# QCDIS/KaFKA-InferenceEngine

Hardware: AMD Instinct MI355X
Metric: pixel-state updates/sec (whole node), 10980^2 S2 tile, 7-param state (higher is better)
Workload: dtype fp32

## Files before the change

csrc/kf_bindings.cpp:

```cpp
#include <pybind11/pybind11.h>
#include <pybind11/stl.h>
#include <stdexcept>
#include <string>
#include <vector>
#include "kf_launch.h"
#include "kf_deflate.h"
#include "kf_inflate.h"
#include "kf_stream.h"

namespace py = pybind11;
using namespace kf;
namespace kf {
void bind_tiff(py::module_& m);
}

template <typename T>
static T* P(uintptr_t v) { return reinterpret_cast<T*>(v); }

static void check_hip(hipError_t e, const char* what) {
  if (e != hipSuccess) throw std::runtime_error(std::string(what) + ": " + hipGetErrorString(e));
}
static void check_host(int rc, const char* what) {
  if (rc != 0) throw std::runtime_error(std::string(what) + ": unsupported n_params on host runner");
}
// ... 87 lines not shown
      .PTR_FIELD(AnalysisArgs, a_out, float*)
      .PTR_FIELD(AnalysisArgs, b_out, float*)
      .PTR_FIELD(AnalysisArgs, a_in, const float*)
      .PTR_FIELD(AnalysisArgs, b_in, const float*)
      .PTR_FIELD(AnalysisArgs, status, uint8_t*)
      .PTR_FIELD(AnalysisArgs, partials, double*)
      .PTR_FIELD(AnalysisArgs, partials_first, double*)
      .PTR_FIELD(AnalysisArgs, order, const int32_t*)
      .def_readwrite("n_visit", &AnalysisArgs::n_visit)
      .PTR_FIELD(AnalysisArgs, n_visit_dev, const int32_t*)
      .PTR_FIELD(AnalysisArgs, dn_out, float*)
      .def_readwrite("a_rows", &AnalysisArgs::a_rows)
      .def_readwrite("dom_check", &AnalysisArgs::dom_check)
      .ARR_FIELD(AnalysisArgs, dom_lo, float)
      .ARR_FIELD(AnalysisArgs, dom_hi, float)
      .def_readwrite("gn_fused", &AnalysisArgs::gn_fused)
      .def_readwrite("band_layout", &AnalysisArgs::band_layout)
      .PTR_FIELD(AnalysisArgs, prop, const PropArgs*)
      .PTR_FIELD(AnalysisArgs, out_mean, float*)
      .PTR_FIELD(AnalysisArgs, out_unc, float*)
      .PTR_FIELD(AnalysisArgs, out_idx, const int64_t*)
      .def_readwrite("out_plane", &AnalysisArgs::out_plane)
      .def_readwrite("reg_gamma", &AnalysisArgs::reg_gamma)
      .def_readwrite("reg_mask", &AnalysisArgs::reg_mask)
      .PTR_FIELD(AnalysisArgs, reg_nbr, const int32_t*)
      .PTR_FIELD(AnalysisArgs, reg_v, float*)
      .PTR_FIELD(AnalysisArgs, x0_out, float*)
      .PTR_FIELD(AnalysisArgs, line_tab, const float*)
      .def_readwrite("line_t0", &AnalysisArgs::line_t0)
      .def_readwrite("line_inv_h", &AnalysisArgs::line_inv_h)
      .def_readwrite("line_n", &AnalysisArgs::line_n)
      .def_readwrite("line_j", &AnalysisArgs::line_j)
      .def_readwrite("a_struct", &AnalysisArgs::a_struct)
      .GEO_FIELDS(AnalysisArgs, reg_geo);

  py::class_<GainArgs>(m, "GainArgs")
      .def(py::init([]() { GainArgs a; memset(&a, 0, sizeof(a)); return a; }))
      .def_readwrite("N", &GainArgs::N)
      .def_readwrite("ld", &GainArgs::ld)
      .def_readwrite("n_bands", &GainArgs::n_bands)
      .def_readwrite("joseph", &GainArgs::joseph)
      .def_readwrite("fast_d", &GainArgs::fast_d)
      .def_readwrite("fast_obs", &GainArgs::fast_obs)
      .def_readwrite("out_plane", &GainArgs::out_plane)
      .def_readwrite("gpm_frags", &GainArgs::gpm_frags)
      .def_readwrite("gpm_global", &GainArgs::gpm_global)
      .def_readwrite("band_layout", &GainArgs::band_layout)
      .def_readwrite("split_mixlo", &GainArgs::split_mixlo)
      .def_readwrite("gn_fused", &GainArgs::gn_fused)
      .def_readwrite("n_visit", &GainArgs::n_visit)
      .PTR_FIELD(GainArgs, n_visit_dev, const int32_t*)
      .def_readwrite("pdiag_rows", &GainArgs::pdiag_rows)
      .PTR_FIELD(GainArgs, partials_first, double*)
      .PTR_FIELD(GainArgs, line_tab, const float*)
      .def_readwrite("line_t0", &GainArgs::line_t0)
      .def_readwrite("line_inv_h", &GainArgs::line_inv_h)
      .def_readwrite("line_n", &GainArgs::line_n)
      .def_readwrite("line_j", &GainArgs::line_j)
      .PTR_FIELD(GainArgs, order, const int32_t*)
      .PTR_FIELD(GainArgs, dn_out, float*)
      .PTR_FIELD(GainArgs, prop, const PropArgs*)
      .PTR_FIELD(GainArgs, out_mean, float*)
      .PTR_FIELD(GainArgs, out_unc, float*)
      .PTR_FIELD(GainArgs, out_idx, const int64_t*)
      .PTR_FIELD(GainArgs, bands, const BandDesc*)
      .PTR_FIELD(GainArgs, x_prev, const float*)
      .PTR_FIELD(GainArgs, x_f, const float*)
// ... 390 lines not shown
```

csrc/kf_core.h:

```cpp
#pragma once
#include <stdint.h>
#include <math.h>

#if defined(__HIPCC__)
#include <hip/hip_runtime.h>
#define KF_HD __host__ __device__ __forceinline__
#else
#define KF_HD inline __attribute__((always_inline))
#endif

enum : int {
  KF_PH_PROLOGUE = 0,
  KF_PH_FORECAST = 1,
  KF_PH_BAND_IN = 2,
  KF_PH_GP = 3,
  KF_PH_BAND_OUT = 4,
  KF_PH_SOLVE = 5,
  KF_PH_GROUPS = 6,
  KF_PH_NSLOT = 8
};
#if defined(KF_PHASE_CLOCKS) && defined(__HIPCC__)
static __device__ unsigned long long kf_phase_clk[KF_PH_NSLOT];
#endif
#if defined(KF_PHASE_CLOCKS) && defined(__HIP_DEVICE_COMPILE__)
// ... 161 lines not shown

KF_HD int32_t geo_neighbour(const StripGeo& g, int64_t N, int64_t p, int k) {
  const uint32_t w = (uint32_t)g.w;
  const uint32_t r = (uint32_t)p / w, c = (uint32_t)p - r * w;
  switch (k) {
    case 0: return r > 0 ? (int32_t)(p - w) : ((g.halo & 1) ? (int32_t)(N + c) : -1);
    case 1: return r + 1 < (uint32_t)g.h ? (int32_t)(p + w) : ((g.halo & 2) ? (int32_t)(N + g.n_up + c) : -1);
    case 2: return c > 0 ? (int32_t)(p - 1) : -1;
    default: return c + 1 < w ? (int32_t)(p + 1) : -1;
  }
}

constexpr int SPEC_ANY = 0, SPEC_PROP = 1, SPEC_PROP_REG = 2;
constexpr int SPEC_PROP_PF = 3;
constexpr int SPEC_PROP_TIP = 4, SPEC_PROP_REG_TIP = 5, SPEC_PROP_PF_TIP = 6;
KF_HD constexpr bool spec_sparse(int spec) { return spec >= SPEC_PROP_TIP; }
KF_HD constexpr int spec_base(int spec) { return spec_sparse(spec) ? spec - 3 : spec; }
constexpr int A_STRUCT_TIP = 1, A_STRUCT_TIP_PRIOR = 2;
template <int SPEC>
struct SpecMask { typedef StructDense type; };
template <> struct SpecMask<SPEC_PROP_TIP> { typedef StructTip type; };
template <> struct SpecMask<SPEC_PROP_REG_TIP> { typedef StructTip type; };
template <> struct SpecMask<SPEC_PROP_PF_TIP> { typedef StructTip type; };

enum AnalysisVariant : int32_t {
  AV_DEFAULT = 0,
  AV_VALU_ORACLE = 4,
  AV_GT_PREFETCH = 7,
  AV_RUNTIME_LAYOUT = 10,
  AV_PER_BAND_OPERAND = 14,
  AV_BLOCK_ORDER = 16,
  AV_GENERIC_SPEC = 18,
  AV_DENSE_SOLVE = 20,
  AV_MIXLO_SPLIT = 22
};

struct AnalysisArgs {
  int64_t N, ld;
  int32_t n_bands, solve;
  int32_t fast_d, fast_obs;
  int32_t variant;
  int32_t gpm_frags;
  int32_t gpm_global;
  const BandDesc* bands;
  const float* x_prev;
  const float* x_f;
  const float* pf_inv;
  float* x_out;
  float* a_out;
  float* b_out;
  const float* a_in;
  const float* b_in;
  uint8_t* status;
  double* partials;
  const PropArgs* prop;
  float* out_mean;
  float* out_unc;
  const int64_t* out_idx;
  int64_t out_plane;
  float reg_gamma;
  uint32_t reg_mask;
  const int32_t* reg_nbr;
  float* reg_v;
  float* x0_out;
  StripGeo reg_geo;
  int32_t gn_fused;
  int32_t band_layout;
  double* partials_first;
  const int32_t* order;
  int64_t n_visit;
  const int32_t* n_visit_dev;
  float* dn_out;
  uint64_t a_rows;
  int32_t dom_check;
  float dom_lo[MAX_D];
  float dom_hi[MAX_D];
  const float* line_tab;
  float line_t0, line_inv_h;
  int32_t line_n, line_j;
  int32_t a_struct;
};

KF_HD int64_t visit_bounded(int64_t n_visit, int64_t N, const int32_t* n_dev) {
  const int64_t n = n_visit > 0 ? n_visit : N;
  if (!n_dev) return n;
  const int64_t d = *n_dev;
  return d < 0 ? 0 : (d < n ? d : n);
}
KF_HD int64_t visit_count(const AnalysisArgs& a) { return visit_bounded(a.n_visit, a.N, a.n_visit_dev); }

template <int NP, typename AP>
KF_HD bool state_out_of_domain(AP a, const float (&x)[NP]) {
  if (!a->dom_check) return false;
  bool o = false;
#pragma unroll
  for (int j = 0; j < NP; ++j) o = o || !(x[j] >= a->dom_lo[j] && x[j] <= a->dom_hi[j]);
  return o;
}
KF_HD bool a_row_on(uint64_t rows, int t) { return rows == 0 || ((rows >> t) & 1u); }



KF_HD int64_t visit_px(const int32_t* order, int64_t q) { return order ? (int64_t)order[q] : q; }
template <int NP>
KF_HD float gather_state(const float (&x)[NP], int idx) {
  float v = x[0];
#pragma unroll
  for (int j = 1; j < NP; ++j) v = (idx == j) ? x[j] : v;
  return v;
}

template <int NP>
KF_HD float gather_state_u(const float (&x)[NP], int idx) {
  float v = x[0];
// ... 1866 lines not shown
```

csrc/kf_device.h:

```cpp
#pragma once
#include <hip/hip_runtime.h>
#include "kf_core.h"
#include "kf_launch.h"
#include "kf_gp_mfma.h"

namespace kf {

constexpr int BLOCK = 256;

__device__ __forceinline__ double wave_sum(double v) {
#pragma unroll
  for (int off = 32; off > 0; off >>= 1) v += __shfl_xor(v, off, 64);
  return v;
}

template <int BS = BLOCK>
__device__ __forceinline__ void block_partial(double v, double* partials) {
  __shared__ double red[BS / 64];
  v = wave_sum(v);
  const int lane = threadIdx.x & 63, wid = threadIdx.x >> 6;
  if (lane == 0) red[wid] = v;
  __syncthreads();
  if (threadIdx.x == 0) {
    double s = 0.0;
// ... 110 lines not shown
  } else {
    for (int64_t base = (int64_t)blockIdx.x * BS + (threadIdx.x - lane); base < nv; base += stride) {
      const int64_t q = base + lane;
      const bool act = q < nv;
      const int64_t p = visit_px(a.order, act ? q : nv - 1);
      float dn1;
      const float dn = pixel_analysis_mfma<NP, D, FOBS, false, false, LAYOUT, IL, SPEC, MIXLO>(a, p, act, gpm_lds,
                                                                                              dn1 KF_PHASE_ARG);
      {
        float* dno = opaque((const KF_CONST_AS AnalysisArgs*)__builtin_amdgcn_kernarg_segment_ptr())->dn_out;
        if (act && dno) KF_PX(dno, 0, p) = dn;
      }
      acc += act ? (double)dn : 0.0;
      acc1 += act ? (double)dn1 : 0.0;
    }
  }
  analysis_partials<BS>(a, acc, acc1);
  KF_PHASE_KERNEL_END
#endif
}

template <int NP, int D, int FOBS, int BS = BLOCK, int MINW = 1, int LAYOUT = BAND_LAYOUT_RUNTIME, bool IL = false,
          int SPEC = SPEC_ANY>
__global__ __launch_bounds__(BS, MINW) void analysis_mfma_kernel(AnalysisArgs a) {
  analysis_mfma_body<NP, D, FOBS, BS, LAYOUT, IL, SPEC, false>(a);
}

template <int NP, int D, int FOBS, int BS = BLOCK, int MINW = 1, int LAYOUT = BAND_LAYOUT_RUNTIME, bool IL = false,
          int SPEC = SPEC_ANY>
__global__ __launch_bounds__(BS, MINW) void analysis_mfma_mixlo_kernel(AnalysisArgs a) {
  analysis_mfma_body<NP, D, FOBS, BS, LAYOUT, IL, SPEC, true>(a);
}

template <int NP, int D, int FOBS, bool PF, bool IL, int SPEC, bool MIXLO>
__device__ __forceinline__ void analysis_mfma_g_body(const AnalysisArgs& a) {
  static_assert(BLOCK / 64 == GPM_G_WAVES, "per-wave LDS transpose buffers of gp_mfma_sums_g_xb");
#if defined(__HIP_DEVICE_COMPILE__)
  KF_PHASE_KERNEL_BEGIN
  double acc = 0.0, acc1 = 0.0;
  const int lane = threadIdx.x & 63;
  const int64_t stride = (int64_t)gridDim.x * BLOCK;
  const int64_t nv = visit_count(a);
  for (int64_t base = (int64_t)blockIdx.x * BLOCK + (threadIdx.x - lane); base < nv; base += stride) {
    const int64_t q = base + lane;
    const bool act = q < nv;
    const int64_t p = visit_px(a.order, act ? q : nv - 1);
    float dn1;
    const float dn = pixel_analysis_mfma<NP, D, FOBS, true, PF, BAND_LAYOUT_RUNTIME, IL, SPEC, MIXLO>(
        a, p, act, nullptr, dn1 KF_PHASE_ARG);
    {
      float* dno = opaque((const KF_CONST_AS AnalysisArgs*)__builtin_amdgcn_kernarg_segment_ptr())->dn_out;
      if (act && dno) KF_PX(dno, 0, p) = dn;
    }
    acc += act ? (double)dn : 0.0;
    acc1 += act ? (double)dn1 : 0.0;
  }
  analysis_partials(a, acc, acc1);
  KF_PHASE_KERNEL_END
#endif
}

template <int NP, int D, int FOBS, bool PF = false, bool IL = false, int SPEC = SPEC_ANY>
__global__ __launch_bounds__(BLOCK, 2) void analysis_mfma_g_kernel(AnalysisArgs a) {
  analysis_mfma_g_body<NP, D, FOBS, PF, IL, SPEC, false>(a);
}

// ... 359 lines not shown
  }
#define KF_MFMA_GO(OBS_, BS_, MINW_, LAY_)                                   \
  {                                                                         \
    if (gpm_il_default<NP, LAY_>() != (a.variant == AV_BLOCK_ORDER))        \
      KF_MFMA_GO1(OBS_, BS_, MINW_, LAY_, true, SPEC_ANY)                   \
    else KF_MFMA_GO1(OBS_, BS_, MINW_, LAY_, false, SPEC_ANY)               \
  }
#define KF_MFMA_GO_SPEC(OBS_, BS_, MINW_, LAY_)                                                      \
  {                                                                                                 \
    constexpr bool IL_ = gpm_il_default<NP, LAY_>();                                                \
    const bool tips = (a.a_struct & A_STRUCT_TIP) && a.variant != AV_DENSE_SOLVE;                   \
    if (a.variant == AV_MIXLO_SPLIT) {     \
      if (!a.prop) KF_MFMA_GO1M(OBS_, BS_, MINW_, LAY_, IL_, SPEC_ANY)                              \
      else if (small) KF_MFMA_GO1M(OBS_, BS_, MINW_, LAY_, IL_, SPEC_PROP_PF_TIP)                   \
      else KF_MFMA_GO1M(OBS_, BS_, MINW_, LAY_, IL_, SPEC_PROP_TIP)                                 \
    }                                                                                               \
    else if (!a.prop || a.variant == AV_BLOCK_ORDER || a.variant == AV_GENERIC_SPEC)                \
      KF_MFMA_GO(OBS_, BS_, MINW_, LAY_)                                                            \
    else if (a.reg_v && tips) KF_MFMA_GO1(OBS_, BS_, MINW_, LAY_, IL_, SPEC_PROP_REG_TIP)          \
    else if (a.reg_v) KF_MFMA_GO1(OBS_, BS_, MINW_, LAY_, IL_, SPEC_PROP_REG)                      \
    else if (small && tips) KF_MFMA_GO1(OBS_, BS_, MINW_, LAY_, IL_, SPEC_PROP_PF_TIP)              \
    else if (small) KF_MFMA_GO1(OBS_, BS_, MINW_, LAY_, IL_, SPEC_PROP_PF)                          \
    else if (tips) KF_MFMA_GO1(OBS_, BS_, MINW_, LAY_, IL_, SPEC_PROP_TIP)                          \
    else KF_MFMA_GO1(OBS_, BS_, MINW_, LAY_, IL_, SPEC_PROP)                                        \
  }
      constexpr int MW = NP <= 7 ? 3 : 1;
      bool tip = false;
      const bool small = a.gpm_frags <= 4 * a.n_bands * gpm_frags_per_chunk(FD) + 1;
      (void)small;
      if constexpr (NP == 7 && FD == 4)
        tip = a.band_layout == BAND_LAYOUT_TIP && a.n_bands == 2 && a.variant != AV_RUNTIME_LAYOUT;
      if (a.fast_obs == OBS_DN16) {
        if constexpr (NP == 7 && FD == 4) {
          if (tip) {
            KF_MFMA_GO_SPEC(OBS_DN16, BLOCK, 3, BAND_LAYOUT_TIP)
            return true;
          }
        }
        KF_MFMA_GO(OBS_DN16, BLOCK, MW, BAND_LAYOUT_RUNTIME)
      } else if (a.fast_obs == OBS_F32) {
        if constexpr (NP == 7 && FD == 4) {
          if (tip) {
            KF_MFMA_GO(OBS_F32, BLOCK, 3, BAND_LAYOUT_TIP)
            return true;
          }
        }
        KF_MFMA_GO(OBS_F32, BLOCK, MW, BAND_LAYOUT_RUNTIME)
      } else {
        return false;
      }
#undef KF_MFMA_GO_SPEC
#undef KF_MFMA_GO
#undef KF_MFMA_GO1
#undef KF_MFMA_GO1M
      return true;
    }
    if constexpr (FD == NP && NP >= 7) {
      if (a.gpm_global && a.variant != AV_VALU_ORACLE) {
        constexpr bool IL = gpm_il_default<NP, BAND_LAYOUT_RUNTIME>();
        if (a.fast_obs == OBS_DN16 && a.variant == AV_GT_PREFETCH)
          launch_tiles(analysis_mfma_g_kernel<NP, FD, OBS_DN16, true>, BLOCK, 0, a, grid, s, n_part);
        else if (NP == 10 && a.fast_obs == OBS_DN16 && a.variant == AV_MIXLO_SPLIT && a.prop && !a.reg_v) {
          if constexpr (NP == 10)
            launch_tiles(analysis_mfma_g_mixlo_kernel<NP, FD, OBS_DN16, false, true, SPEC_PROP>, BLOCK, 0, a, grid, s,
                         n_part);
        } else if (NP == 10 && a.fast_obs == OBS_DN16 && a.variant == AV_MIXLO_SPLIT) {
// ... 60 lines not shown
```

csrc/kf_gp_mfma.h:

```cpp
#pragma once
#include <hip/hip_runtime.h>
#include <type_traits>
#include "kf_core.h"

namespace kf {

typedef _Float16 kf_h8 __attribute__((ext_vector_type(8)));
typedef float kf_f16v __attribute__((ext_vector_type(16)));
typedef uint32_t kf_u4 __attribute__((ext_vector_type(4)));
typedef __fp16 kf_hp2 __attribute__((ext_vector_type(2)));

KF_HD constexpr int gpm_k_steps(int D) { return (3 * D + 2 + 15) / 16; }
KF_HD constexpr int gpm_lo_row(int D) { return D + 1 <= 8 ? 8 : 16; }
KF_HD constexpr int gpm_sum_rows(int D) { return 2 * (D + 1); }
KF_HD constexpr int gpm_frags_per_chunk(int D) { return 64 * gpm_k_steps(D) + 4 * gpm_sum_rows(D); }
constexpr int GPM_MAX_D = 10;
constexpr int GPM_MAX_BANDS = 4;
constexpr int GPM_G_WAVES = 4;

#if defined(__HIP_DEVICE_COMPILE__)
__device__ __forceinline__ uint32_t gpm_pack(_Float16 a, _Float16 b) {
  return (uint32_t)__builtin_bit_cast(uint16_t, a) | ((uint32_t)__builtin_bit_cast(uint16_t, b) << 16);
}

// ... 649 lines not shown
          if (ka->a_out) store_a_rows<NP, M>(ka, p, A);
#pragma unroll
          for (int j = 0; j < NP; ++j) KF_PXS(ka->x_out, j * ld, p) = x1[j];
          if (ka->out_unc) {
            const int64_t r = ka->out_idx ? KF_PXS(ka->out_idx, 0, p) : p;
            const int64_t pl = ka->out_plane;
            if (ka->out_mean) {
#pragma unroll
              for (int j = 0; j < NP; ++j) KF_PXS(ka->out_mean, j * pl, r) = x1[j];
            }
#pragma unroll
            for (int j = 0; j < NP; ++j) KF_PXS(ka->out_unc, j * pl, r) = kf_rsqrt(A[tri(NP, j, j)]);
          }
          if (ka->status) KF_PXS(ka->status, 0, p) = st;
        }
        KF_PHASE(KF_PH_SOLVE)
        return 0.f;
      }
    }
  }
  if (!SPARSE || it + 1 >= ka->gn_fused) {
    if (state_out_of_domain<NP>(ka, x0)) st |= ST_OUT_OF_DOMAIN;
  }
  const bool last = it + 1 >= ka->gn_fused;
  const float dn = analysis_epilogue<NP, true, SPEC>(ka, p, A, b, x0, st, last && act, last);
  KF_PHASE(KF_PH_SOLVE)
  if (last) return act ? dn : 0.f;
  dn_first = dn;
#pragma unroll
  for (int j = 0; j < NP; ++j) x0[j] = b[j];
  }
}

template <int NP, int D, int FOBS, bool GT = false, bool IL = false, bool MIXLO = false>
__device__ __forceinline__ float pixel_gain_mfma(const GainArgs& a, int64_t p, bool act, const kf_h8* lds,
                                                 float& dn1) {
  constexpr bool SXC = GT && D == NP && D % 2 == 0;
  kf_h8 sxb[2][gpm_k_steps(D)];
  int sx_it = -1;
  return gain_pixel<NP>(a, p, act, dn1, [&](int bi, int it, const float (&x0)[NP], float& y, float& w, float& H0,
                                            float (&h)[NP], bool& ok) -> bool {
    int off = 0;
    if constexpr (!GT)
      for (int bj = 0; bj < bi; ++bj) off += cptr(a.bands)[bj].gpm_nchunk * gpm_frags_per_chunk(D);
    const KF_CONST_AS BandDesc* bdp = cptr(a.bands) + bi;
    decode_obs<FOBS>(*bdp, p, y, w);
    const bool use = act && (w > 0.f);
    H0 = 0.f;
#pragma unroll
    for (int j = 0; j < NP; ++j) h[j] = 0.f;
    ok = false;
    const int nch = bdp->gpm_nchunk;
    bool tabled = false;
    const KF_CONST_AS GainArgs* la = opaque((const KF_CONST_AS GainArgs*)__builtin_amdgcn_kernarg_segment_ptr());
    if (it == 0 && !a.x_prev && la->line_tab && __any(use)) {
      const LinePos lp = line_pos<NP>(la, x0, a.n_bands * (D + 1) * 4);
      if (__all(lp.in || !use)) {
        float g[D];
        line_eval<D>(lp.row + bi * (D + 1) * 4, lp.s, H0, g);
        const KF_CONST_AS BandDesc* q = opaque(bdp);
        if (q->map_identity) {
#pragma unroll
          for (int d = 0; d < D && d < NP; ++d) h[d] = g[d];
        } else {
#pragma unroll
          for (int d = 0; d < D; ++d) {
// ... 57 lines not shown
```

kafka_inferenceengine_amd/ops/kernels.py:

```python
from __future__ import annotations

import itertools
from dataclasses import dataclass
from enum import IntEnum

import numpy as np
import torch

from ..models.gp import gpm_frags_per_chunk
from ..utils.blocks import ntri
from . import _ext

OBS_NONE, OBS_F32, OBS_DN16, OBS_BF16, OBS_BF16Y = 0, 1, 2, 3, 4
ST_NONSPD, ST_NONFINITE, ST_BAD_OP, ST_NO_OBS, ST_FALLBACK, ST_OUT_OF_DOMAIN = 1, 2, 4, 8, 16, 32
SUPPORTED_NP = (1, 2, 3, 4, 7, 10)


def ext():
    return _ext.require_ext()


def _ptr(t):
    return 0 if t is None else int(t.data_ptr())

# ... 57 lines not shown

def check_np(n_params: int):
    if n_params not in SUPPORTED_NP:
        raise ValueError(f"n_params={n_params} has no compiled kernel (supported: {SUPPORTED_NP}); "
                         "pad the state (engine.padding) to a supported size")


def grid_for(N: int) -> int:
    return int(ext().grid(int(N)))


def partials_buffer(N: int, device) -> torch.Tensor:
    return torch.zeros(grid_for(N), dtype=torch.float64, device=device)


def _set_valid(partials, n):
    if partials is not None:
        partials._kf_n = int(n)


@dataclass
class BandTable:
    buf: torch.Tensor
    n: int
    keepalive: tuple
    fast_d: int = 0
    fast_obs: int = 0
    gpm_frags: int = 0
    gpm_global: bool = False
    layout: int = 0
    dom: tuple | None = None
    specs: tuple = ()
    tip_maps: bool = False

    @property
    def ptr(self) -> int:
        return int(self.buf.data_ptr())


OP_PRECOMP = 0
OP_LINEAR = 1
OP_GP = 2


GPM_MAX_LDS = 160 * 1024
GPM_MAX_BANDS = 4
GPM_GLOBAL_D = (7, 10)
GAIN_GLOBAL_D = (10,)

BAND_LAYOUT_TIP = 1
BAND_LAYOUT_SHARED_X = 2
FD_PRECOMP = -1
FD_LINEAR = -2


class Variant(IntEnum):
    DEFAULT = 0
    VALU_ORACLE = 4
    GT_PREFETCH = 7
    RUNTIME_LAYOUT = 10
    PER_BAND_OPERAND = 14
    BLOCK_ORDER = 16
    GENERIC_SPEC = 18
    DENSE_SOLVE = 20
    MIXLO_SPLIT = 22


DEFAULT_VARIANT = Variant.DEFAULT


class _PinnedRing:

    SLOT = 16 << 10
    SLOTS = 64

    def __init__(self, device):
        self.device = device
        self.buf = torch.empty(self.SLOT * self.SLOTS, dtype=torch.uint8, pin_memory=True)
        self.events = [None] * self.SLOTS
        self.i = 0

    def copy(self, cpu: torch.Tensor) -> torch.Tensor:
        n = cpu.numel() * cpu.element_size()
        j = self.i
        self.i = (self.i + 1) % self.SLOTS
        if self.events[j] is not None:
            self.events[j].synchronize()
        stage = self.buf[j * self.SLOT:j * self.SLOT + n]
        stage.copy_(cpu.reshape(-1).view(torch.uint8))
        out = torch.empty(n, dtype=torch.uint8, device=self.device)
        out.copy_(stage, non_blocking=True)
        ev = torch.cuda.Event()
        ev.record(torch.cuda.current_stream(self.device))
        self.events[j] = ev
        return out.view(cpu.dtype).view(cpu.shape)


_RINGS = {}
# ... 12 lines not shown
        return ring.copy(cpu)
    return cpu.pin_memory().to(device, non_blocking=True)


def make_band_table(descs: list, device, keepalive=(), specs=()) -> BandTable:
    raw = ext().pack_band_descs(descs)
    cpu = torch.frombuffer(bytearray(raw), dtype=torch.uint8) if raw else torch.zeros(8, dtype=torch.uint8)
    buf = small_h2d(cpu, device)
    fast_d = fast_obs = 0
    obs = {d.obs for d in descs}
    one_obs = next(iter(obs)) if len(obs) == 1 else None
    if descs and all(d.op == OP_GP for d in descs):
        ds = {d.d for d in descs}
        if len(ds) == 1 and one_obs in (OBS_F32, OBS_DN16):
            fast_d, fast_obs = next(iter(ds)), one_obs
    elif descs and one_obs in (OBS_F32, OBS_DN16, OBS_BF16, OBS_BF16Y) and all(d.op == OP_PRECOMP for d in descs):
        fast_d, fast_obs = FD_PRECOMP, one_obs
    elif descs and one_obs in (OBS_F32, OBS_DN16, OBS_BF16, OBS_BF16Y) and all(d.op == OP_LINEAR for d in descs):
        fast_d, fast_obs = FD_LINEAR, one_obs
    gpm_frags, gpm_global = 0, False
    if fast_d > 0 and all(d.gpm_nchunk > 0 for d in descs):
        gpm_frags = sum(d.gpm_nchunk for d in descs) * gpm_frags_per_chunk(fast_d) + 1
        if gpm_frags * 16 > GPM_MAX_LDS or len(descs) > GPM_MAX_BANDS:
            gpm_frags, gpm_global = 0, fast_d in GPM_GLOBAL_D
    layout = 0
    if fast_d == 4 and gpm_frags > 0 and [d.map_kind for d in descs] == [2, 3]:
        layout = BAND_LAYOUT_TIP
    elif (gpm_global and fast_d % 2 == 0 and all(d.map_identity for d in descs)
          and len({tuple(d.center[:fast_d]) for d in descs}) == 1):
        layout = BAND_LAYOUT_SHARED_X
    tip_maps = len(descs) == 2 and all(d.op == OP_GP and d.d == 4 for d in descs) and \
        [d.map_kind for d in descs] == [2, 3]
    return BandTable(buf, len(descs), tuple(keepalive), fast_d, fast_obs, gpm_frags, gpm_global, layout,
                     _state_domain(descs), tuple(specs), tip_maps)


def _state_domain(descs):
    lo, hi, any_ = [-np.inf] * 16, [np.inf] * 16, False
    for d in descs:
        if d.op != OP_GP or not d.dom_check:
            continue
        m, c, dl, dh = d.map, d.center, d.dom_lo, d.dom_hi
        for i in range(int(d.d)):
            j = int(m[i])
            lo[j] = max(lo[j], float(dl[i]) + float(c[i]))
            hi[j] = min(hi[j], float(dh[i]) + float(c[i]))
            any_ = True
    return (lo, hi) if any_ else None


LINE_TABLES = True
_LINE_CACHE: dict = {}


def _prop_single(mask: int):
    mask = int(mask)
    if mask == 0:
        return -1
    return mask.bit_length() - 1 if mask & (mask - 1) == 0 else None


def line_fields(bands: BandTable, prop, n_params: int, dev):
    if dev.type != "cuda" or prop is None or bands.fast_d <= 0 or not bands.specs or \
            not (bands.gpm_frags > 0 or bands.gpm_global):
        return None
    if any(getattr(sp, "kind", None) != OP_GP or len(sp.state_map) != bands.fast_d for sp in bands.specs):
        return None
    j = _prop_single(prop.args.prop_mask)
    if j is None:
        return None
    fixed = tuple(float(v) for v in list(prop.args.reset_mean)[:n_params])
    key = (tuple(id(sp) for sp in bands.specs), fixed, j, dev)
    hit = _LINE_CACHE.get(key)
    if hit is None:
        from ..models.gp import line_table

        r = line_table(list(bands.specs), np.asarray(fixed, dtype=np.float64), j)
        tab = None if r is None else torch.from_numpy(np.ascontiguousarray(r[0])).to(dev)
        if len(_LINE_CACHE) >= 32:
            _LINE_CACHE.clear()
        hit = _LINE_CACHE[key] = (bands.specs, None if r is None else (tab, r[1], r[2], r[3], j))
    return hit[1]


def _set_line(a, bands, prop, n_params, dev, x_prev, line):
    if x_prev is not None or not (LINE_TABLES if line is None else line):
        return
    lf = line_fields(bands, prop, n_params, dev)
    if lf is not None:
        a.line_tab, a.line_t0, a.line_inv_h, a.line_n, a.line_j = _ptr(lf[0]), lf[1], lf[2], lf[3], lf[4]


A_STRUCT_TIP = 1
A_STRUCT_TIP_PRIOR = 2
TIP_ZERO_ENTRIES = ((0, 3), (0, 4), (0, 5), (1, 3), (1, 4), (1, 5), (2, 3), (2, 4))
STRUCT_LAUNCHES = {"tip": 0, "dense": 0}


def _tri(n, i, j):
    return i * n - (i * (i - 1)) // 2 + (j - i)


def tip_structure(n_params, bands: BandTable, prop, variant=None) -> int:
    v = DEFAULT_VARIANT if variant is None else variant
    if prop is None or n_params != 7 or not bands.tip_maps or int(v) not in (int(Variant.DEFAULT),
                                                                             int(Variant.MIXLO_SPLIT)):
        return 0
    c = [float(x) for x in list(prop.args.reset_cinv)[:ntri(7)]]
    if any(c[_tri(7, i, j)] != 0.0 for i, j in TIP_ZERO_ENTRIES):
        return 0
    flags = A_STRUCT_TIP
    off = [c[_tri(7, i, j)] for i in range(7) for j in range(i + 1, 7) if (i, j) != (2, 5)]
    mean = [float(x) for x in list(prop.args.reset_mean)[:7]]
    if all(x == 0.0 for x in off) and all(np.isfinite(x) for x in c) and all(np.isfinite(x) for x in mean):
        flags |= A_STRUCT_TIP_PRIOR
    return flags


def gp_operator(n_params, bands: BandTable, x, h0, h, N=None, d=None):
    check_np(n_params)
    N = int(x.shape[1] if N is None else N)
    _check_soa(x, n_params, N, "x")
    nb = bands.n
    d = bands.fast_d if d is None else d
    if h0.shape[0] != nb or h.shape[0] != nb * n_params or h0.shape[1] != h.shape[1] or h0.shape[1] < N:
        raise ValueError("h0 must be [nb, ldh] and h [nb*n_params, ldh]")
    if _dev(x) and not ext().gp_operator_supported(n_params, int(d)):
        raise ValueError(f"no gp_operator kernel for n_params={n_params}, d={d}")
    ext().gp_operator(n_params, int(d), bands.ptr, nb, _ptr(x), N, x.shape[1], _ptr(h0), _ptr(h), h0.shape[1],
                      _dev(x), _stream(x))


def gp_operator_supported(n_params, d) -> bool:
    return bool(ext().gp_operator_supported(int(n_params), int(d)))


def analysis(n_params, bands: BandTable, x_prev, x_f, pf_inv, x_out=None, a_out=None, b_out=None, status=None,
             partials=None, N=None, solve=True, fast=True, variant=None, a_in=None, b_in=None, prop=None,
             out=None, reg=None, x0_out=None, gn_fused=1, partials_first=None, order=None, n_visit=None,
             dn_out=None, a_rows=None, n_visit_dev=None, line=None):
    ref = next(t for t in (x_prev, x_f, x_out, a_out) if t is not None)
    key = None
    if reg is None:
        key = (n_params, _table_key(bands), N, bool(solve), bool(fast),
               DEFAULT_VARIANT if variant is None else variant, gn_fused, n_visit, _sig(n_visit_dev), a_rows,
               None if prop is None else (prop.device_copy().data_ptr(), prop.args.ld, prop.args.N, prop.fused,
                                          prop.device),
               _sig(x_prev), _sig(x_f), _sig(pf_inv), _sig(x_out), _sig(a_out), _sig(b_out), _sig(status),
               _sig(partials), _sig(a_in), _sig(b_in), _sig(x0_out), _sig(partials_first), _sig(order), _sig(dn_out),
               None if out is None else (_sig(out[0]), _sig(out[1]), _sig(out[2])),
               LINE_TABLES if line is None else bool(line))
        hit = _ANALYSIS_MEMO.get(key)
        if hit is not None:
            a, grid = hit
            if a.prop:
                STRUCT_LAUNCHES["tip" if getattr(a, "a_struct", 0) else "dense"] += 1
            n_part = ext().analysis(n_params, a, grid, _dev(ref), _stream(ref))
            _set_valid(partials, n_part)
            _set_valid(partials_first if gn_fused == 2 else None, n_part)
            return partials
    check_np(n_params)
    N = int(ref.shape[1] if N is None else N)
    dev = ref.device
    nt = ntri(n_params)
    if prop is None and (x_prev is None or x_f is None or pf_inv is None):
        raise ValueError("x_prev, x_f and pf_inv are required unless the propagation is fused")
    if prop is not None and (x_f is not None or pf_inv is not None or a_in is not None):
        raise ValueError("fused propagation replaces x_f/pf_inv and excludes a_in")
    for t, r, nm in ((x_prev, n_params, "x_prev"), (x_f, n_params, "x_f"), (pf_inv, nt, "pf_inv"),
                     (x_out, n_params, "x_out"), (a_out, nt, "a_out"), (b_out, n_params, "b_out")):
        _check_soa(t, r, N, nm, device=dev)
    ld = ref.shape[1]
    for t in (x_prev, x_f, pf_inv, x_out, a_out, b_out):
        if t is not None and t.shape[1] != ld:
            raise ValueError("all SoA operands must share the leading dimension")
    if prop is not None and (prop.args.ld != ld or prop.args.N < N or prop.device != dev):
        raise ValueError("fused propagation arguments do not match the analysis layout/device")
    if prop is not None and not prop.fused:
        raise ValueError("analysis(prop=...) needs prop_args(..., fused=True)")
    if solve and x_out is None:
        raise ValueError("solve=True needs x_out")
    _check_vec(status, N, "status", torch.uint8, dev)
    if partials is not None and (partials.dtype != torch.float64 or partials.numel() < grid_for(N)):
        raise ValueError("partials must be float64 with >= grid_for(N) entries")
    if gn_fused not in (1, 2):
        raise ValueError("gn_fused must be 1 or 2")
    if gn_fused == 2 and (a_in is not None or not solve):
        raise ValueError("gn_fused=2 runs the solve path only (no band chunks or solve=False)")
    if gn_fused == 2 and reg is not None and x0_out is None:
# ... 63 lines not shown
                raise ValueError(f"dense geometry {geo} does not cover N={N} pixels")
            a.geo_w, a.geo_h, a.geo_halo, a.geo_n_up = int(geo["w"]), int(geo["h"]), int(geo["halo"]), \
                int(geo["n_up"])
    if order is not None:
        _check_vec(order, N, "order", torch.int32, dev)
        a.order = _ptr(order)
    nv = N
    if n_visit is not None:
        nv = int(n_visit)
        if order is None or not 0 < nv <= N:
            raise ValueError(f"n_visit={n_visit} needs an order and 0 < n_visit <= N={N}")
        if gn_fused != 1 or reg is not None:
            raise ValueError("n_visit: single-iteration launches without the regulariser")
        a.n_visit = nv
    if n_visit_dev is not None:
        if n_visit is None:
            raise ValueError("n_visit_dev needs n_visit (the bound that sizes the grid)")
        _check_vec(n_visit_dev, 1, "n_visit_dev", torch.int32, dev)
        a.n_visit_dev = _ptr(n_visit_dev)
    if dn_out is not None:
        _check_vec(dn_out, N, "dn_out", torch.float32, dev)
        a.dn_out = _ptr(dn_out)
    if bands.dom is not None:
        a.dom_check, a.dom_lo, a.dom_hi = 1, list(bands.dom[0]), list(bands.dom[1])
    if a_rows:
        if int(a_rows) >> nt:
            raise ValueError(f"a_rows has bits past the {nt} packed rows")
        a.a_rows = int(a_rows)
    if fast:
        _set_line(a, bands, prop, n_params, dev, x_prev, line)
    if prop is not None and a_in is None and hasattr(a, "a_struct") and (
            dev.type != "cuda" or (fast and a.band_layout == BAND_LAYOUT_TIP and bands.fast_obs == OBS_DN16)):
        a.a_struct = tip_structure(n_params, bands, prop, v)
    if prop is not None:
        STRUCT_LAUNCHES["tip" if getattr(a, "a_struct", 0) else "dense"] += 1
    grid = grid_for(nv)
    if partials is not None and partials.numel() < grid:
        raise ValueError("partials must hold one entry per workgroup (partials_buffer)")
    n_part = ext().analysis(n_params, a, grid, _dev(ref), _stream(ref))
    if key is not None:
        if len(_ANALYSIS_MEMO) >= 64:
            _ANALYSIS_MEMO.clear()
        _ANALYSIS_MEMO[key] = (a, grid)
    _set_valid(partials, n_part)
    _set_valid(partials_first if gn_fused == 2 else None, n_part)
    return partials


CHUNK_GROUP_RUNS = 16


def chunk_groups(lc_ptr) -> int:
    runs = np.diff(np.asarray(lc_ptr, dtype=np.int64))
    return max(1, int(-(-runs.max() // CHUNK_GROUP_RUNS))) if runs.size else 1


def chunk_partials(dn, seg_start, seg_len, lc_ptr, lc_gid, active, part, gpart, groups, qinv, clamp):
    n_local = int(lc_gid.numel())
    if gpart.numel() < n_local * groups or gpart.dtype != torch.int64 or part.dtype != torch.int64:
        raise ValueError("chunk_partials: int64 part / group scratch of the right size")
    if qinv.dtype != torch.float64 or qinv.numel() != part.numel():
        raise ValueError("chunk_partials: qinv must be float64 [nc]")
    ext().chunk_partials(_ptr(dn), _ptr(seg_start), _ptr(seg_len), _ptr(lc_ptr), _ptr(lc_gid), n_local,
                         _ptr(active), _ptr(part), _ptr(gpart), int(groups), _ptr(qinv), int(clamp), _dev(part),
                         _stream(part))


def chunk_decide(part_all, world, len_x, local_count, tol, n_iter, min_iter, max_iter, active, newly, iters, info,
# ... 723 lines not shown
```

Baseline: 5.762 billion.

## Add straight-line specialized tip analysis kernel with precomputed constant block

New measurement: 6.043 billion, median of 6. 4.9% higher.

```diff
diff --git a/csrc/kf_bindings.cpp b/csrc/kf_bindings.cpp
--- a/csrc/kf_bindings.cpp
+++ b/csrc/kf_bindings.cpp
@@ -143,7 +143,63 @@
       .def_readwrite("line_n", &AnalysisArgs::line_n)
       .def_readwrite("line_j", &AnalysisArgs::line_j)
       .def_readwrite("a_struct", &AnalysisArgs::a_struct)
+      .def_property_readonly("tc_on", [](const AnalysisArgs& s) { return s.tc.on != 0; })
+      .def_property_readonly("tc", [](const AnalysisArgs& s) {
+        const TipConst& t = s.tc;
+        py::dict d;
+        d["on"] = t.on;
+        d["j"] = t.j;
+        d["m"] = t.m;
+        d["q"] = t.q;
+        d["xa_row"] = (uintptr_t)t.xa_row;
+        d["pa_row"] = (uintptr_t)t.pa_row;
+        d["dn"] = std::vector<uintptr_t>{(uintptr_t)t.dn[0], (uintptr_t)t.dn[1]};
+        d["line_tab"] = (uintptr_t)t.line_tab;
+        d["line_t0"] = t.line_t0;
+        d["line_inv_h"] = t.line_inv_h;
+        d["line_n"] = t.line_n;
+        d["dom_check"] = t.dom_check;
+        d["dom_lo"] = get_arr(t.dom_lo);
+        d["dom_hi"] = get_arr(t.dom_hi);
+        d["mean"] = get_arr(t.mean);
+        d["cinv"] = get_arr(t.cinv);
+        py::list bands;
+        for (int b = 0; b < 2; ++b) {
+          const TipBandConst& c = t.band[b];
+          py::dict e;
+          e["center"] = get_arr(c.center);
+          e["coef"] = get_arr(c.coef);
+          e["offset"] = c.offset;
+          e["gpm_scale"] = c.gpm_scale;
+          e["scale"] = c.scale;
+          e["rel_unc"] = c.rel_unc;
+          e["unc_floor"] = c.unc_floor;
+          e["nchunk"] = c.nchunk;
+          bands.append(e);
+        }
+        d["band"] = bands;
+        d["rows"] = t.rows;
+        d["out"] = t.out;
+        d["ld"] = t.ld;
+        d["out_plane"] = t.out_plane;
+        d["x_out"] = (uintptr_t)t.x_out;
+        d["a_out"] = (uintptr_t)t.a_out;
+        d["out_mean"] = (uintptr_t)t.out_mean;
+        d["out_unc"] = (uintptr_t)t.out_unc;
+        d["out_idx"] = (uintptr_t)t.out_idx;
+        d["status"] = (uintptr_t)t.status;
+        d["gn_fused"] = t.gn_fused;
+        d["gpm_frags"] = t.gpm_frags;
+        return d;
+      })
       .GEO_FIELDS(AnalysisArgs, reg_geo);
+
+  m.def("tip_sl_shape", [](int np, const AnalysisArgs& a, const PropArgs* pa, const std::vector<BandDesc>& bd) {
+    return tip_sl_shape(np, a, pa, bd.data(), (int)bd.size());
+  });
+  m.def("tip_const_fill", [](int np, AnalysisArgs& a, const PropArgs* pa, const std::vector<BandDesc>& bd) {
+    return tip_const_fill(np, a, pa, bd.data(), (int)bd.size());
+  });
 
   py::class_<GainArgs>(m, "GainArgs")
       .def(py::init([]() { GainArgs a; memset(&a, 0, sizeof(a)); return a; }))
diff --git a/csrc/kf_core.h b/csrc/kf_core.h
--- a/csrc/kf_core.h
+++ b/csrc/kf_core.h
@@ -217,7 +217,43 @@
   AV_BLOCK_ORDER = 16,
   AV_GENERIC_SPEC = 18,
   AV_DENSE_SOLVE = 20,
-  AV_MIXLO_SPLIT = 22
+  AV_MIXLO_SPLIT = 22,
+  AV_LOOPED_TIP = 24
+};
+
+struct TipBandConst {
+  float center[4], coef[4];
+  float offset, gpm_scale;
+  float scale, rel_unc, unc_floor;
+  int32_t nchunk;
+  int32_t pad[2];
+};
+constexpr int TIP_ROWS_NONE = 0, TIP_ROWS_DIAG = 1, TIP_ROWS_ALL = 2;
+constexpr int TIP_OUT_NONE = 0, TIP_OUT_UNC = 1, TIP_OUT_MEAN = 2;
+struct TipConst {
+  int32_t on;
+  int32_t j;
+  float m, q;
+  const float* xa_row;
+  const float* pa_row;
+  const uint16_t* dn[2];
+  const float* line_tab;
+  float line_t0, line_inv_h;
+  int32_t line_n;
+  int32_t dom_check;
+  float dom_lo[8], dom_hi[8];
+  float mean[8];
+  float cinv[28];
+  TipBandConst band[2];
+  int32_t rows, out;
+  int64_t ld, out_plane;
+  float* x_out;
+  float* a_out;
+  float* out_mean;
+  float* out_unc;
+  const int64_t* out_idx;
+  uint8_t* status;
+  int32_t gn_fused, gpm_frags;
 };
 
 struct AnalysisArgs {
@@ -264,7 +300,86 @@
   float line_t0, line_inv_h;
   int32_t line_n, line_j;
   int32_t a_struct;
+  TipConst tc;
 };
+
+KF_HD int prop_single(uint32_t mask);
+inline bool tip_sl_shape(int np, const AnalysisArgs& a, const PropArgs* pa, const BandDesc* bd, int nb) {
+  if (np != 7 || !pa || !bd || nb != 2 || a.n_bands != 2) return false;
+  if (a.variant != AV_DEFAULT) return false;
+  if (a.fast_d != 4 || a.fast_obs != OBS_DN16 || a.band_layout != BAND_LAYOUT_TIP) return false;
+  if (a.gpm_frags <= 0 || a.gpm_global) return false;
+  if (!a.prop || a.x_prev || a.x_f || a.pf_inv || a.a_in || a.b_in) return false;
+  if ((a.a_struct & (A_STRUCT_TIP | A_STRUCT_TIP_PRIOR)) != (A_STRUCT_TIP | A_STRUCT_TIP_PRIOR)) return false;
+  if (!a.solve || !a.x_out || a.b_out || a.x0_out || a.reg_v) return false;
+  if (a.gn_fused != 1 && a.gn_fused != 2) return false;
+  if (a.out_mean && !a.out_unc) return false;
+  const int j = prop_single(pa->prop_mask);
+  if (pa->mode != PROP_PRIOR_PARTIAL || pa->blend || j < 0 || j >= 7 || pa->q_pix || !pa->x_a || !pa->p_a) return false;
+  if (pa->ld != a.ld) return false;
+  if (a.line_tab && a.line_j != j) return false;
+  for (int b = 0; b < 2; ++b) {
+    const BandDesc& d = bd[b];
+    if (d.op != OP_GP || d.obs != OBS_DN16 || d.d != 4 || !d.dn || d.h0_out || d.gpm_nchunk < 1) return false;
+    if (d.map_kind != (b == 0 ? GPM_MAP_TIP_VIS : GPM_MAP_TIP_NIR)) return false;
+  }
+  if (a.a_out && a.a_rows != 0 && a.a_rows != (1ull << tri(7, j, j))) return false;
+  const int64_t lim = (int64_t)1 << 30;
+  if (a.N < 1 || a.N > a.ld || a.ld >= lim || (a.out_unc && (a.out_plane < 1 || a.out_plane >= lim))) return false;
+  if (a.out_idx && a.N >= lim / 2) return false;
+  return true;
+}
+
+inline bool tip_const_fill(int np, AnalysisArgs& a, const PropArgs* pa, const BandDesc* bd, int nb) {
+  TipConst& t = a.tc;
+  t = TipConst{};
+  if (!tip_sl_shape(np, a, pa, bd, nb)) return false;
+  t.on = 1;
+  t.j = prop_single(pa->prop_mask);
+  t.m = pa->m[t.j];
+  t.q = pa->q[t.j];
+  t.xa_row = pa->x_a + (int64_t)t.j * pa->ld;
+  t.pa_row = pa->p_a + (int64_t)tri(7, t.j, t.j) * pa->ld;
+  t.line_tab = a.line_tab;
+  t.line_t0 = a.line_t0;
+  t.line_inv_h = a.line_inv_h;
+  t.line_n = a.line_n;
+  t.dom_check = a.dom_check;
+  for (int i = 0; i < 7; ++i) {
+    t.dom_lo[i] = a.dom_lo[i];
+    t.dom_hi[i] = a.dom_hi[i];
+    t.mean[i] = pa->reset_mean[i];
+  }
+  for (int i = 0; i < 28; ++i) t.cinv[i] = pa->reset_cinv[i];
+  for (int b = 0; b < 2; ++b) {
+    const BandDesc& d = bd[b];
+    TipBandConst& c = t.band[b];
+    for (int i = 0; i < 4; ++i) {
+      c.center[i] = d.center[i];
+      c.coef[i] = d.coef[i];
+    }
+    c.offset = d.offset;
+    c.gpm_scale = d.gpm_scale;
+    c.scale = d.scale;
+    c.rel_unc = d.rel_unc;
+    c.unc_floor = d.unc_floor;
+    c.nchunk = d.gpm_nchunk;
+    t.dn[b] = d.dn;
+  }
+  t.rows = !a.a_out ? TIP_ROWS_NONE : (a.a_rows ? TIP_ROWS_DIAG : TIP_ROWS_ALL);
+  t.out = !a.out_unc ? TIP_OUT_NONE : (a.out_mean ? TIP_OUT_MEAN : TIP_OUT_UNC);
+  t.ld = a.ld;
+  t.out_plane = a.out_plane;
+  t.x_out = a.x_out;
+  t.a_out = a.a_out;
+  t.out_mean = a.out_mean;
+  t.out_unc = a.out_unc;
+  t.out_idx = a.out_idx;
+  t.status = a.status;
+  t.gn_fused = a.gn_fused;
+  t.gpm_frags = a.gpm_frags;
+  return true;
+}
 
 KF_HD int64_t visit_bounded(int64_t n_visit, int64_t N, const int32_t* n_dev) {
   const int64_t n = n_visit > 0 ? n_visit : N;
diff --git a/csrc/kf_device.h b/csrc/kf_device.h
--- a/csrc/kf_device.h
+++ b/csrc/kf_device.h
@@ -166,6 +166,79 @@
   analysis_mfma_body<NP, D, FOBS, BS, LAYOUT, IL, SPEC, true>(a);
 }
 
+template <bool IL, int ROWS, int OUT>
+__global__ __launch_bounds__(BLOCK, 3) void analysis_tip_sl_kernel(AnalysisArgs a) {
+#if defined(__HIP_DEVICE_COMPILE__)
+  extern __shared__ kf_h8 gpm_lds[];
+  KF_PHASE_KERNEL_BEGIN
+  {
+    int off = 0;
+#pragma unroll
+    for (int bi = 0; bi < 2; ++bi) {
+      const KF_CONST_AS BandDesc* bd = cptr(a.bands) + bi;
+      const int n = bd->gpm_nchunk * gpm_frags_per_chunk(4);
+      const kf_h8* src = (const kf_h8*)bd->gpm;
+      for (int i = threadIdx.x; i < n; i += BLOCK) gpm_lds[off + i] = src[i];
+      off += n;
+    }
+    if (threadIdx.x == 0) gpm_lds[a.gpm_frags - 1] = kf_h8{};
+  }
+  __syncthreads();
+  KF_PHASE(KF_PH_PROLOGUE)
+  double acc = 0.0, acc1 = 0.0;
+  const int lane = threadIdx.x & 63;
+  const int64_t stride = (int64_t)gridDim.x * BLOCK;
+  const int64_t nv = visit_count(a);
+  for (int64_t base = (int64_t)blockIdx.x * BLOCK + (threadIdx.x - lane); base < nv; base += stride) {
+    const int64_t q = base + lane;
+    const bool act = q < nv;
+    const int64_t p = visit_px(a.order, act ? q : nv - 1);
+    const KF_CONST_AS AnalysisArgs* ka = opaque((const KF_CONST_AS AnalysisArgs*)__builtin_amdgcn_kernarg_segment_ptr());
+    const TipGroup g = tip_group_load<OUT>(&ka->tc, p);
+    float dn1;
+    const float dn = pixel_analysis_tip_sl<IL, ROWS, OUT>(p, act, g, gpm_lds, dn1 KF_PHASE_ARG);
+    {
+      float* dno = opaque((const KF_CONST_AS AnalysisArgs*)__builtin_amdgcn_kernarg_segment_ptr())->dn_out;
+      if (act && dno) KF_PX(dno, 0, p) = dn;
+    }
+    acc += act ? (double)dn : 0.0;
+    acc1 += act ? (double)dn1 : 0.0;
+  }
+  analysis_partials<BLOCK>(a, acc, acc1);
+  KF_PHASE_KERNEL_END
+#endif
+}
+
+template <typename K>
+static void gpm_lds_attr(K kernel, size_t bytes);
+
+template <int ROWS, int OUT>
+static void launch_tip_sl(size_t lds, const AnalysisArgs& a, int grid, hipStream_t s, int* n_part) {
+  constexpr bool IL = true;
+  gpm_lds_attr(analysis_tip_sl_kernel<IL, ROWS, OUT>, lds);
+  *n_part = grid;
+  hipLaunchKernelGGL((analysis_tip_sl_kernel<IL, ROWS, OUT>), dim3(grid), dim3(BLOCK), lds, s, a);
+}
+
+static bool l_analysis_tip_sl(size_t lds, const AnalysisArgs& a, int grid, hipStream_t s, int* n_part) {
+#define KF_TIP_SL_GO(R_, O_)                               \
+  if (a.tc.rows == R_ && a.tc.out == O_) {                 \
+    launch_tip_sl<R_, O_>(lds, a, grid, s, n_part);        \
+    return true;                                           \
+  }
+  KF_TIP_SL_GO(TIP_ROWS_NONE, TIP_OUT_NONE)
+  KF_TIP_SL_GO(TIP_ROWS_NONE, TIP_OUT_UNC)
+  KF_TIP_SL_GO(TIP_ROWS_NONE, TIP_OUT_MEAN)
+  KF_TIP_SL_GO(TIP_ROWS_DIAG, TIP_OUT_NONE)
+  KF_TIP_SL_GO(TIP_ROWS_DIAG, TIP_OUT_UNC)
+  KF_TIP_SL_GO(TIP_ROWS_DIAG, TIP_OUT_MEAN)
+  KF_TIP_SL_GO(TIP_ROWS_ALL, TIP_OUT_NONE)
+  KF_TIP_SL_GO(TIP_ROWS_ALL, TIP_OUT_UNC)
+  KF_TIP_SL_GO(TIP_ROWS_ALL, TIP_OUT_MEAN)
+#undef KF_TIP_SL_GO
+  return false;
+}
+
 template <int NP, int D, int FOBS, bool PF, bool IL, int SPEC, bool MIXLO>
 __device__ __forceinline__ void analysis_mfma_g_body(const AnalysisArgs& a) {
   static_assert(BLOCK / 64 == GPM_G_WAVES, "per-wave LDS transpose buffers of gp_mfma_sums_g_xb");
@@ -591,6 +664,7 @@
         tip = a.band_layout == BAND_LAYOUT_TIP && a.n_bands == 2 && a.variant != AV_RUNTIME_LAYOUT;
       if (a.fast_obs == OBS_DN16) {
         if constexpr (NP == 7 && FD == 4) {
+          if (tip && a.tc.on && a.variant == AV_DEFAULT && l_analysis_tip_sl(lds, a, grid, s, n_part)) return true;
           if (tip) {
             KF_MFMA_GO_SPEC(OBS_DN16, BLOCK, 3, BAND_LAYOUT_TIP)
             return true;
diff --git a/csrc/kf_gp_mfma.h b/csrc/kf_gp_mfma.h
--- a/csrc/kf_gp_mfma.h
+++ b/csrc/kf_gp_mfma.h
@@ -705,6 +705,284 @@
   }
 }
 
+struct TipGroup {
+  float xa, pa;
+  uint16_t dn[2];
+  uint32_t r;
+};
+
+template <int OUT>
+__device__ __forceinline__ TipGroup tip_group_load(const KF_CONST_AS TipConst* tc, int64_t p) {
+  TipGroup g;
+  g.xa = KF_PXS(tc->xa_row, 0, p);
+  g.pa = KF_PXS(tc->pa_row, 0, p);
+  g.dn[0] = KF_PXS(tc->dn[0], 0, p);
+  g.dn[1] = KF_PXS(tc->dn[1], 0, p);
+  g.r = (uint32_t)p;
+  if constexpr (OUT != TIP_OUT_NONE) {
+    const int64_t* oi = tc->out_idx;
+    if (oi) g.r = (uint32_t)KF_PXS(oi, 0, p);
+  }
+  return g;
+}
+
+__device__ __forceinline__ float tip_forecast(const KF_CONST_AS TipConst* tc, float xa, float pa, float (&xf)[7],
+                                              float (&P)[28]) {
+#pragma unroll
+  for (int i = 0; i < 7; ++i)
+#pragma unroll
+    for (int j = i; j < 7; ++j)
+      if (StructTip::on(i, j)) P[tri(7, i, j)] = tc->cinv[tri(7, i, j)];
+  const int J = tc->j;
+  const float pjj = kf_rcp(kf_rcp(pa) + tc->q);
+  const float xj = tc->m * xa;
+#pragma unroll
+  for (int j = 0; j < 7; ++j) {
+    P[tri(7, j, j)] = (j == J) ? pjj : P[tri(7, j, j)];
+    xf[j] = (j == J) ? xj : tc->mean[j];
+  }
+  return pjj;
+}
+
+template <int ROWS>
+__device__ __forceinline__ void tip_store_rows(const KF_CONST_AS TipConst* tc, int64_t p, const float (&A)[28]) {
+  if constexpr (ROWS == TIP_ROWS_ALL) {
+    const int64_t ld = tc->ld;
+#pragma unroll
+    for (int i = 0; i < 7; ++i)
+#pragma unroll
+      for (int j = i; j < 7; ++j) {
+        const int t = tri(7, i, j);
+        if (StructTip::on(i, j)) KF_PXS(tc->a_out, t * ld, p) = A[t];
+        else KF_PXS(tc->a_out, t * ld, p) = tc->cinv[t];
+      }
+  } else if constexpr (ROWS == TIP_ROWS_DIAG) {
+    const int J = tc->j;
+    float dg[7];
+#pragma unroll
+    for (int j = 0; j < 7; ++j) dg[j] = A[tri(7, j, j)];
+    const float v = gather_state_u<7>(dg, J);
+    KF_PXS(tc->a_out, (int64_t)(J * 7 - (J * (J - 1)) / 2) * tc->ld, p) = v;
+  }
+}
+
+template <int K>
+__device__ __forceinline__ void tip_inputs(const KF_CONST_AS TipBandConst* bc, const float (&x0)[7], float (&xi)[4],
+                                           float& c) {
+  constexpr GpmMap M = gpm_const_map(K);
+#pragma unroll
+  for (int d = 0; d < 4; ++d) xi[d] = x0[M.m[d]] - bc->center[d];
+#pragma unroll
+  for (int d = 0; d < 4; ++d) c = fmaf(bc->coef[d] * xi[d], xi[d], c);
+}
+
+template <bool IL, int ROWS, int OUT>
+__device__ __forceinline__ float pixel_analysis_tip_sl(int64_t p, bool act, const TipGroup& grp, const kf_h8* lds,
+                                                       float& dn_first KF_PHASE_PARAM) {
+  constexpr int NP = 7, D = 4, NT = 28;
+  typedef StructTip M;
+  float x0[NP], A[NT], b[NP];
+  dn_first = 0.f;
+  KF_PHASE_COUNT(KF_PH_GROUPS)
+  for (int it = 0;; ++it) {
+    p = opaque_lane(p);
+    const KF_CONST_AS TipConst* tc =
+        &opaque((const KF_CONST_AS AnalysisArgs*)__builtin_amdgcn_kernarg_segment_ptr())->tc;
+    uint8_t st = 0;
+    {
+      float xf[NP];
+      const float pjj = tip_forecast(tc, grp.xa, grp.pa, xf, A);
+      if (!((pjj > 0.f) && finitef(pjj))) st |= ST_NONSPD;
+      if (it == 0) {
+#pragma unroll
+        for (int j = 0; j < NP; ++j) {
+          x0[j] = xf[j];
+          b[j] = 0.f;
+        }
+      } else {
+        prior_rhs<NP, true, M>(A, xf, x0, b);
+      }
+    }
+    int nobs = 0;
+    int off = 0;
+    bool wave_obs = false;
+    const bool line = it == 0 && tc->line_tab;
+    LinePos lp_it{nullptr, 0.f, false};
+    if (line) {
+      const int n = tc->line_n;
+      const float t = gather_state_u<NP>(x0, tc->j);
+      const float u = (t - tc->line_t0) * tc->line_inv_h;
+      lp_it.in = u >= 0.f && u <= (float)n;
+      const float uc = fminf(fmaxf(u, 0.f), (float)n);
+      const int k = min((int)uc, n - 1);
+      lp_it.s = uc - (float)k;
+      lp_it.row = tc->line_tab + (int64_t)k * (2 * (D + 1) * 4);
+    }
+    auto band = [&](auto bic, auto mkc) {
+      constexpr int BI = decltype(bic)::value, MK = decltype(mkc)::value;
+      const KF_CONST_AS TipBandConst* bc = &tc->band[BI];
+      float y, w;
+      {
+        const uint16_t dn = grp.dn[BI];
+        const float yd = (float)dn * bc->scale;
+        const float sig = fmaxf(bc->rel_unc * yd, bc->unc_floor);
+        const bool okd = dn > 0 && sig > 0.f;
+        w = okd ? kf_rcp(sig * sig) : 0.f;
+        y = dn > 0 ? yd : 0.f;
+      }
+      const bool use = act && (w > 0.f);
+      float H0 = 0.f, g[D];
+#pragma unroll
+      for (int d = 0; d < D; ++d) g[d] = 0.f;
+      bool ok = false;
+      const int nch = bc->nchunk;
+      const bool any = __any(use);
+      wave_obs = wave_obs || any;
+      bool tabled = false;
+      if (any && line) {
+        if (__all(lp_it.in || !use)) {
+          line_eval<D>(lp_it.row + BI * (D + 1) * 4, lp_it.s, H0, g);
+          tabled = true;
+          ok = true;
+        }
+      }
+      if (any && !tabled) {
+        float xi[D], c = 0.f;
+        tip_inputs<MK>(bc, x0, xi, c);
+        c *= -0.5f * LOG2E;
+        float S[D + 1];
+        KF_PHASE(KF_PH_BAND_IN)
+        gp_mfma_sums<D, IL, false>(lds + off, lds + tc->gpm_frags - 1, nch, xi, c, S);
+        KF_PHASE(KF_PH_GP)
+        const KF_CONST_AS TipBandConst* q = opaque(bc);
+        const float sc = q->gpm_scale;
+        const float S0 = S[0] * sc;
+        H0 = q->offset + S0;
+#pragma unroll
+        for (int d = 0; d < D; ++d) g[d] = fmaf(-q->coef[d] * xi[d], S0, LN2 * (S[1 + d] * sc));
+        ok = finitef(H0);
+#pragma unroll
+        for (int d = 0; d < D; ++d) ok = ok && finitef(g[d]);
+      }
+      off += nch * gpm_frags_per_chunk(D);
+      if (use && !ok) st |= ST_BAD_OP;
+      if (use && ok) {
+        ++nobs;
+        const float wy = w * (y - H0);
+        gpm_update_const<NP, D, MK>(A, b, g, w, wy);
+      }
+      KF_PHASE(KF_PH_BAND_OUT)
+    };
+    KF_PHASE(KF_PH_FORECAST)
+    band(std::integral_constant<int, 0>{}, std::integral_constant<int, GPM_MAP_TIP_VIS>{});
+    band(std::integral_constant<int, 1>{}, std::integral_constant<int, GPM_MAP_TIP_NIR>{});
+    if (nobs == 0) st |= ST_NO_OBS;
+    const KF_CONST_AS TipConst* ka =
+        &opaque((const KF_CONST_AS AnalysisArgs*)__builtin_amdgcn_kernarg_segment_ptr())->tc;
+    const int64_t ld = ka->ld;
+    auto out_of_domain = [&](const float (&x)[NP]) {
+      bool o = false;
+#pragma unroll
+      for (int j = 0; j < NP; ++j) o = o || !(x[j] >= ka->dom_lo[j] && x[j] <= ka->dom_hi[j]);
+      return ka->dom_check && o;
+    };
+    auto store_out = [&](const float (&x)[NP], const float (&dA)[NP]) {
+      if constexpr (OUT != TIP_OUT_NONE) {
+        const int64_t r = (int64_t)grp.r;
+        const int64_t pl = ka->out_plane;
+        if constexpr (OUT == TIP_OUT_MEAN) {
+#pragma unroll
+          for (int j = 0; j < NP; ++j) KF_PXS(ka->out_mean, j * pl, r) = x[j];
+        }
+#pragma unroll
+        for (int j = 0; j < NP; ++j) KF_PXS(ka->out_unc, j * pl, r) = kf_rsqrt(dA[j]);
+      }
+    };
+    if (it == 0 && !wave_obs) {
+      bool healthy = true;
+#pragma unroll
+      for (int j = 0; j < NP; ++j) {
+        float s = A[tri(NP, j, j)];
+        if (j == 5) {
+          const float s2 = A[tri(NP, 2, 2)];
+          const float u25 = A[tri(NP, 2, 5)] * kf_rsqrt(s2 > 0.f ? s2 : 1.f);
+          s = fmaf(-u25, u25, s);
+        }
+        healthy = healthy && (s > 0.f) && finitef(s) && finitef(x0[j]);
+      }
+      if (__all(healthy)) {
+        st = ST_NO_OBS;
+        float x1[NP];
+#pragma unroll
+        for (int j = 0; j < NP; ++j) x1[j] = x0[j] + 0.f;
+        if (out_of_domain(x1)) st |= ST_OUT_OF_DOMAIN;
+        if (act) {
+          tip_store_rows<ROWS>(ka, p, A);
+#pragma unroll
+          for (int j = 0; j < NP; ++j) KF_PXS(ka->x_out, j * ld, p) = x1[j];
+          float dA[NP];
+#pragma unroll
+          for (int j = 0; j < NP; ++j) dA[j] = A[tri(NP, j, j)];
+          store_out(x1, dA);
+          uint8_t* sp = ka->status;
+          if (sp) KF_PXS(sp, 0, p) = st;
+        }
+        KF_PHASE(KF_PH_SOLVE)
+        return 0.f;
+      }
+    }
+    const bool last = it + 1 >= ka->gn_fused;
+    if (last) {
+      if (out_of_domain(x0)) st |= ST_OUT_OF_DOMAIN;
+    }
+    const bool store = last && act;
+    if (store) tip_store_rows<ROWS>(ka, p, A);
+    float dn = 0.f;
+    {
+      float dA[NP];
+#pragma unroll
+      for (int j = 0; j < NP; ++j) dA[j] = A[tri(NP, j, j)];
+      const bool spd = chol_packed<NP, M>(A) && !(st & ST_NONSPD);
+      chol_solve<NP, M>(A, b);
+      {
+#pragma clang fp contract(off)
+#pragma unroll
+        for (int j = 0; j < NP; ++j) b[j] = b[j] + x0[j];
+      }
+      bool fin = true;
+#pragma unroll
+      for (int j = 0; j < NP; ++j) fin = fin && finitef(b[j]);
+      if (!spd || !fin) {
+        st |= (!spd ? ST_NONSPD : 0) | (!fin ? ST_NONFINITE : 0) | ST_FALLBACK;
+        tip_forecast(opaque(ka), grp.xa, grp.pa, b, A);
+#pragma unroll
+        for (int j = 0; j < NP; ++j) dA[j] = A[tri(NP, j, j)];
+        if (store) tip_store_rows<ROWS>(ka, p, A);
+      }
+      if (store) {
+#pragma unroll
+        for (int j = 0; j < NP; ++j) KF_PXS(ka->x_out, j * ld, p) = b[j];
+      }
+#pragma unroll
+      for (int j = 0; j < NP; ++j) {
+        const float d = b[j] - x0[j];
+        dn = fmaf(d, d, dn);
+      }
+      if ((st & ST_FALLBACK) && !finitef(dn)) dn = 0.f;
+      if (store) {
+        store_out(b, dA);
+        uint8_t* sp = ka->status;
+        if (sp) KF_PXS(sp, 0, p) = st;
+      }
+    }
+    KF_PHASE(KF_PH_SOLVE)
+    if (last) return act ? dn : 0.f;
+    dn_first = dn;
+#pragma unroll
+    for (int j = 0; j < NP; ++j) x0[j] = b[j];
+  }
+}
+
 template <int NP, int D, int FOBS, bool GT = false, bool IL = false, bool MIXLO = false>
 __device__ __forceinline__ float pixel_gain_mfma(const GainArgs& a, int64_t p, bool act, const kf_h8* lds,
                                                  float& dn1) {
diff --git a/kafka_inferenceengine_amd/ops/kernels.py b/kafka_inferenceengine_amd/ops/kernels.py
--- a/kafka_inferenceengine_amd/ops/kernels.py
+++ b/kafka_inferenceengine_amd/ops/kernels.py
@@ -113,6 +113,7 @@
     dom: tuple | None = None
     specs: tuple = ()
     tip_maps: bool = False
+    descs: tuple = ()
 
     @property
     def ptr(self) -> int:
@@ -145,6 +146,7 @@
     GENERIC_SPEC = 18
     DENSE_SOLVE = 20
     MIXLO_SPLIT = 22
+    LOOPED_TIP = 24
 
 
 DEFAULT_VARIANT = Variant.DEFAULT
@@ -223,7 +225,7 @@
     tip_maps = len(descs) == 2 and all(d.op == OP_GP and d.d == 4 for d in descs) and \
         [d.map_kind for d in descs] == [2, 3]
     return BandTable(buf, len(descs), tuple(keepalive), fast_d, fast_obs, gpm_frags, gpm_global, layout,
-                     _state_domain(descs), tuple(specs), tip_maps)
+                     _state_domain(descs), tuple(specs), tip_maps, tuple(descs))
 
 
 def _state_domain(descs):
@@ -286,6 +288,15 @@
 A_STRUCT_TIP_PRIOR = 2
 TIP_ZERO_ENTRIES = ((0, 3), (0, 4), (0, 5), (1, 3), (1, 4), (1, 5), (2, 3), (2, 4))
 STRUCT_LAUNCHES = {"tip": 0, "dense": 0}
+TIP_SL_LAUNCHES = {"straight": 0, "looped": 0}
+
+
+def _count_launch(a):
+    if a.prop:
+        tip = bool(getattr(a, "a_struct", 0))
+        STRUCT_LAUNCHES["tip" if tip else "dense"] += 1
+        if tip:
+            TIP_SL_LAUNCHES["straight" if getattr(a, "tc_on", False) else "looped"] += 1
 
 
 def _tri(n, i, j):
@@ -294,8 +305,8 @@
 
 def tip_structure(n_params, bands: BandTable, prop, variant=None) -> int:
     v = DEFAULT_VARIANT if variant is None else variant
-    if prop is None or n_params != 7 or not bands.tip_maps or int(v) not in (int(Variant.DEFAULT),
-                                                                             int(Variant.MIXLO_SPLIT)):
+    if prop is None or n_params != 7 or not bands.tip_maps or int(v) not in (
+            int(Variant.DEFAULT), int(Variant.MIXLO_SPLIT), int(Variant.LOOPED_TIP)):
         return 0
     c = [float(x) for x in list(prop.args.reset_cinv)[:ntri(7)]]
     if any(c[_tri(7, i, j)] != 0.0 for i, j in TIP_ZERO_ENTRIES):
@@ -344,8 +355,7 @@
         hit = _ANALYSIS_MEMO.get(key)
         if hit is not None:
             a, grid = hit
-            if a.prop:
-                STRUCT_LAUNCHES["tip" if getattr(a, "a_struct", 0) else "dense"] += 1
+            _count_launch(a)
             n_part = ext().analysis(n_params, a, grid, _dev(ref), _stream(ref))
             _set_valid(partials, n_part)
             _set_valid(partials_first if gn_fused == 2 else None, n_part)
@@ -475,8 +485,9 @@
     if prop is not None and a_in is None and hasattr(a, "a_struct") and (
             dev.type != "cuda" or (fast and a.band_layout == BAND_LAYOUT_TIP and bands.fast_obs == OBS_DN16)):
         a.a_struct = tip_structure(n_params, bands, prop, v)
-    if prop is not None:
-        STRUCT_LAUNCHES["tip" if getattr(a, "a_struct", 0) else "dense"] += 1
+    if dev.type == "cuda" and prop is not None and getattr(a, "a_struct", 0) and hasattr(ext(), "tip_const_fill"):
+        ext().tip_const_fill(n_params, a, prop.args, list(bands.descs))
+    _count_launch(a)
     grid = grid_for(nv)
     if partials is not None and partials.numel() < grid:
         raise ValueError("partials must hold one entry per workgroup (partials_buffer)")
```
